# happyxtt/CNNs_SLFP_quantization

Hardware: AMD Instinct MI355X
Metric: images/sec at batch 256, MobileNetV1 SLFP<3,4> ImageNet-224; % HBM roofline (higher is better)
Workload: dtype f32 (1x1 contraction: fp16 MFMA operands, f32 accumulate); 1 GPU; mobilenetv1_imagenet224: all 27 Conv2d_Q layers, SLFP<3,4> Qbits=8, NHWC, batch 256 per GPU as 2 concurrent image groups of 128 on 2 HIP streams, inputs resident in HBM; batch_per_gpu=256, global_batch=256, parallelism=batch-sharded x1, one-time RCCL broadcast of the u8 weight codes, pointwise_mfma=pw_mfma_f16x1

## Files before the change

### cnns_slfp_quantization_amd/_lib.py

```python
import ctypes
import os

_HERE = os.path.dirname(os.path.abspath(__file__))
LIB_PATH = os.path.join(_HERE, "libslfp_hip.so")

OK, ERR_BAD_ARG, ERR_SHAPE, ERR_UNSUPPORTED, ERR_ALIGNMENT, ERR_HIP = 0, -1, -2, -3, -4, -5
FMT_ACT8, FMT_W8, FMT_SFP7, FMT_EXT = 0, 1, 2, 4
LAYOUT_NCHW, LAYOUT_NHWC = 0, 1
BWD_DENSE = 1
MFMA_DEFAULT, MFMA_F16X1, MFMA_F16X3 = 0, 1, 3
OPT_SGD, OPT_DSGD, OPT_SSGD = 0, 1, 2
LAYEROUT_LUT_BYTES = 4928

SYMBOLS = (
    "slfp_version", "slfp_last_error", "slfp_device_count",
    "slfp_encode_f32", "slfp_decode_f32", "slfp_quantize_f32", "slfp_quantize_layerout_f32", "slfp_absmax_f32",
    "slfp_conv2d_out_shape", "slfp_conv2d_kernel_name", "slfp_conv2d_wprep_bytes",
    "slfp_conv2d_prepare_weights", "slfp_conv2d_prepare_weights_codes", "slfp_conv2d_workspace_bytes", "slfp_conv2d_fwd", "slfp_conv2d_fwd_post",
    "slfp_linear_workspace_bytes", "slfp_linear_fwd", "slfp_linear_prepare_weights", "slfp_linear_fwd_prepared",
    "slfp_nchw_to_nhwc_f32", "slfp_nhwc_to_nchw_f32", "slfp_debug_div_mismatches",
    "slfp_debug_enc_mismatches", "slfp_enc_table_ok", "slfp_dwpw_supported", "slfp_dwpw_fwd",
    "slfp_conv2d_codes_supported", "slfp_conv2d_fwd_codes", "slfp_conv2d_fwd_codes_ws", "slfp_maxpool2d_codes", "slfp_debug_code_mismatches", "slfp_debug_reload_switches",
    "slfp_debug_enc_hl_mismatches", "slfp_sgd_step_f32", "slfp_debug_dw3x3_variant", "slfp_debug_dense_variant", "slfp_debug_pw_variant",
    "slfp_conv2d_bwd_supported", "slfp_conv2d_bwd_kernel_name", "slfp_conv2d_bwd_workspace_bytes", "slfp_conv2d_bwd",
    "slfp_conv2d_bwd_supported_ex", "slfp_conv2d_bwd_kernel_name_ex", "slfp_conv2d_bwd_workspace_bytes_ex", "slfp_conv2d_bwd_ex",
    "slfp_conv2d_res_supported", "slfp_conv2d_fwd_res",
    "slfp_conv2d_codes_slice_supported", "slfp_conv2d_fwd_codes_slice", "slfp_maxpool2d_codes_ex", "slfp_maxpool2d_out_shape",
    "slfp_conv2d_entry_supported", "slfp_conv2d_fwd_entry",
    "slfp_conv2d_res_codes_supported", "slfp_conv2d_fwd_res_codes",
    "slfp_layerout_lut_classes", "slfp_layerout_lut_values", "slfp_layerout_lut_index", "slfp_conv2d_codes_lut_supported",
    "slfp_conv2d_fwd_codes_lut", "slfp_debug_layerout_lut_mismatches",
    "slfp_dwpw_codes_supported", "slfp_dwpw_fwd_codes",
    "slfp_linear_fc_supported", "slfp_linear_fc_workspace_bytes", "slfp_linear_fwd_fc", "slfp_debug_linear_fc_tiles",
    "slfp_global_avgpool_supported", "slfp_global_avgpool_f32",
    "slfp_debug_dw3x3_instance", "slfp_debug_code_relu_mismatches",
    "slfp_bn_train_supported", "slfp_bn_train_workspace_bytes", "slfp_bn_train_fwd", "slfp_bn_train_bwd", "slfp_debug_bn_split",
    "slfp_debug_dwpw_instance",
)


class ConvDesc(ctypes.Structure):
    _fields_ = [
        ("n", ctypes.c_int64), ("c_in", ctypes.c_int64), ("h", ctypes.c_int64), ("w", ctypes.c_int64),
        ("c_out", ctypes.c_int64), ("kh", ctypes.c_int64), ("kw", ctypes.c_int64),
        ("stride_h", ctypes.c_int32), ("stride_w", ctypes.c_int32), ("pad_h", ctypes.c_int32),
        ("pad_w", ctypes.c_int32), ("dil_h", ctypes.c_int32), ("dil_w", ctypes.c_int32),
        ("groups", ctypes.c_int32), ("x_layout", ctypes.c_int32), ("y_layout", ctypes.c_int32),
        ("qbits", ctypes.c_int32), ("ka", ctypes.c_float), ("kw_scale", ctypes.c_float),
        ("mfma_passes", ctypes.c_int32), ("reserved", ctypes.c_int32),
    ]


class ConvIo(ctypes.Structure):
    _fields_ = [("x_codes", ctypes.c_int32), ("y_codes", ctypes.c_int32), ("y_ka", ctypes.c_float), ("y_qbits", ctypes.c_int32)]


class SgdHparams(ctypes.Structure):
    _fields_ = [("rule", ctypes.c_int32), ("qbits", ctypes.c_int32), ("lr", ctypes.c_float), ("momentum", ctypes.c_float),
                ("damp_alpha", ctypes.c_float), ("weight_decay", ctypes.c_float), ("nesterov", ctypes.c_int32),
                ("reserved", ctypes.c_int32)]


class SlfpError(RuntimeError):
    def __init__(self, code, text):
        super().__init__(f"libslfp_hip: {text} (status {code})")
        self.code = code


_lib = None


def load():
    global _lib
    if _lib is not None:
        return _lib
    if not os.path.exists(LIB_PATH):
        raise RuntimeError(
            f"{LIB_PATH} is missing: the SLFP HIP extension is not built. "
            "Run `python -m cnns_slfp_quantization_amd.build` (needs hipcc). There is no CPU fallback.")
    import torch
    L = ctypes.CDLL(LIB_PATH)
    vp, sz, ci, cf, i64 = ctypes.c_void_p, ctypes.c_size_t, ctypes.c_int, ctypes.c_float, ctypes.c_int64
    dp = ctypes.POINTER(ConvDesc)
    sigs = {
        "slfp_version": (ci, []),
        "slfp_last_error": (ctypes.c_char_p, []),
        "slfp_device_count": (ci, []),
        "slfp_encode_f32": (ci, [vp, vp, sz, cf, ci, vp]),
        "slfp_decode_f32": (ci, [vp, vp, sz, ci, vp]),
        "slfp_quantize_f32": (ci, [vp, vp, sz, cf, ci, vp]),
        "slfp_quantize_layerout_f32": (ci, [vp, vp, sz, vp]),
        "slfp_absmax_f32": (ci, [vp, sz, vp, vp]),
        "slfp_conv2d_out_shape": (ci, [dp, ctypes.POINTER(i64), ctypes.POINTER(i64)]),
        "slfp_conv2d_kernel_name": (ctypes.c_char_p, [dp]),
        "slfp_debug_dw3x3_variant": (ctypes.c_char_p, [dp, ci]),
        "slfp_debug_dw3x3_instance": (ctypes.c_char_p, [dp, ctypes.POINTER(ConvIo), ci, ci, ci]),
        "slfp_debug_code_relu_mismatches": (ci, [cf, ci, vp, vp]),
        "slfp_debug_dense_variant": (ctypes.c_char_p, [dp, ci]),
        "slfp_debug_pw_variant": (ctypes.c_char_p, [dp, ctypes.POINTER(ConvIo), ci, ci, i64]),
        "slfp_conv2d_wprep_bytes": (sz, [dp]),
        "slfp_conv2d_prepare_weights": (ci, [dp, vp, vp, vp, vp]),
        "slfp_conv2d_prepare_weights_codes": (ci, [dp, vp, vp, vp, vp]),
        "slfp_conv2d_workspace_bytes": (sz, [dp]),
        "slfp_conv2d_fwd": (ci, [dp, vp, vp, vp, vp, vp, vp, vp]),
        "slfp_conv2d_fwd_post": (ci, [dp, vp, vp, vp, vp, vp, ci, vp, vp, vp, vp]),
        "slfp_linear_workspace_bytes": (sz, [i64, i64, i64]),
        "slfp_linear_fwd": (ci, [vp, vp, vp, vp, i64, i64, i64, cf, cf, ci, ci, vp, vp]),
        "slfp_linear_prepare_weights": (ci, [vp, vp, i64, i64, cf, ci, ci, vp]),
        "slfp_linear_fwd_prepared": (ci, [vp, vp, vp, vp, i64, i64, i64, cf, cf, ci, ci, vp]),
        "slfp_nchw_to_nhwc_f32": (ci, [vp, vp, i64, i64, i64, i64, vp]),
        "slfp_nhwc_to_nchw_f32": (ci, [vp, vp, i64, i64, i64, i64, vp]),
        "slfp_debug_div_mismatches": (ci, [cf, vp, vp]),
        "slfp_debug_enc_mismatches": (ci, [cf, ci, vp, vp]),
        "slfp_enc_table_ok": (ci, [cf, ci]),
        "slfp_dwpw_supported": (ci, [dp, dp]),
        "slfp_dwpw_fwd": (ci, [dp, dp, vp, vp, vp, vp, ci, vp, vp, vp, vp, ci, vp, vp]),
        "slfp_conv2d_codes_supported": (ci, [dp, ctypes.POINTER(ConvIo), ci, ci]),
        "slfp_conv2d_fwd_codes": (ci, [dp, ctypes.POINTER(ConvIo), vp, vp, vp, vp, vp, ci, vp, vp]),
        "slfp_conv2d_fwd_codes_ws": (ci, [dp, ctypes.POINTER(ConvIo), vp, vp, vp, vp, vp, ci, vp, vp, vp]),
        "slfp_maxpool2d_codes": (ci, [vp, vp, i64, i64, i64, i64, ci, ci, ci, ci, ci, ci, ci, vp]),
        "slfp_debug_code_mismatches": (ci, [cf, ci, vp, vp]),
        "slfp_debug_reload_switches": (None, []),
        "slfp_debug_enc_hl_mismatches": (ci, [cf, ci, vp, vp]),
        "slfp_sgd_step_f32": (ci, [ctypes.POINTER(SgdHparams), sz, vp, vp, vp, vp, vp, vp]),
        "slfp_conv2d_bwd_supported": (ci, [dp]),
        "slfp_conv2d_bwd_kernel_name": (ctypes.c_char_p, [dp]),
        "slfp_conv2d_bwd_workspace_bytes": (sz, [dp, ci, ci]),
        "slfp_conv2d_bwd": (ci, [dp, vp, vp, vp, vp, vp, vp, vp, vp]),
        "slfp_conv2d_bwd_supported_ex": (ci, [dp, ctypes.c_uint]),
        "slfp_conv2d_bwd_kernel_name_ex": (ctypes.c_char_p, [dp, ctypes.c_uint]),
        "slfp_conv2d_bwd_workspace_bytes_ex": (sz, [dp, ctypes.c_uint, ci, ci]),
        "slfp_conv2d_bwd_ex": (ci, [dp, ctypes.c_uint, vp, vp, vp, vp, vp, vp, vp, vp]),
        "slfp_conv2d_res_supported": (ci, [dp, ctypes.POINTER(ConvIo), ci, ci]),
        "slfp_conv2d_fwd_res": (ci, [dp, ctypes.POINTER(ConvIo), vp, vp, vp, vp, vp, ci, vp, vp, vp, vp]),
        "slfp_conv2d_codes_slice_supported": (ci, [dp, ctypes.POINTER(ConvIo), ci, ci, i64]),
        "slfp_conv2d_fwd_codes_slice": (ci, [dp, ctypes.POINTER(ConvIo), vp, vp, vp, vp, vp, ci, vp, i64, vp, vp]),
        "slfp_maxpool2d_codes_ex": (ci, [vp, vp, i64, i64, i64, i64, ci, ci, ci, ci, ci, ci, ci, ci, vp]),
        "slfp_maxpool2d_out_shape": (ci, [i64, i64, ci, ci, ci, ci, ci, ci, ci, ctypes.POINTER(i64), ctypes.POINTER(i64)]),
        "slfp_conv2d_entry_supported": (ci, [dp, ctypes.POINTER(ConvIo), ci, ci]),
        "slfp_conv2d_fwd_entry": (ci, [dp, ctypes.POINTER(ConvIo), vp, vp, vp, vp, vp, ci, vp, vp]),
        "slfp_conv2d_res_codes_supported": (ci, [dp, ctypes.POINTER(ConvIo), ci, ci]),
        "slfp_conv2d_fwd_res_codes": (ci, [dp, ctypes.POINTER(ConvIo), vp, vp, vp, vp, vp, ci, vp, vp, vp, vp, vp]),
        "slfp_layerout_lut_classes": (ci, []),
        "slfp_layerout_lut_values": (ci, [vp, ci]),
        "slfp_layerout_lut_index": (ci, [cf]),
        "slfp_conv2d_codes_lut_supported": (ci, [dp, ctypes.POINTER(ConvIo), ci, i64]),
        "slfp_conv2d_fwd_codes_lut": (ci, [dp, ctypes.POINTER(ConvIo), vp, vp, vp, vp, vp, vp, vp, i64, vp, vp]),
        "slfp_debug_layerout_lut_mismatches": (ci, [vp, vp]),
# ... 36 lines not shown
```

### cnns_slfp_quantization_amd/csrc/codec.hip

```cpp
#include <cstdarg>
#include <mutex>
#include <map>
#include <set>
#include <utility>
#include <cstdio>
#include "slfp_device.hpp"
#include "slfp_enc.hpp"
#include "slfp_host.hpp"

namespace slfp {

static thread_local char g_err[512] = "";

void set_error(const char* fmt, ...) {
    va_list ap;
    va_start(ap, fmt);
    vsnprintf(g_err, sizeof(g_err), fmt, ap);
    va_end(ap);
}

int fail(int code, const char* fmt, ...) {
    va_list ap;
    va_start(ap, fmt);
    vsnprintf(g_err, sizeof(g_err), fmt, ap);
    va_end(ap);
    return code;
}

int check_launch(const char* what) {
    hipError_t e = hipGetLastError();
    if (e != hipSuccess) return fail(SLFP_ERR_HIP, "%s: %s", what, hipGetErrorString(e));
    return SLFP_OK;
}

const char* last_error_text() { return g_err; }

int raise_lds_limit(const void* fn, size_t lds_bytes) {
    if (lds_bytes <= 48 * 1024) return SLFP_OK;
    static std::mutex mu;
    static std::map<std::pair<int, const void*>, size_t> raised;
    int dev = 0;
    if (hipGetDevice(&dev) != hipSuccess) return check_launch("hipGetDevice");
    std::lock_guard<std::mutex> lock(mu);
    const auto key = std::make_pair(dev, fn);
    const auto it = raised.find(key);
    if (it != raised.end() && it->second >= lds_bytes) return SLFP_OK;
    if (hipFuncSetAttribute(fn, hipFuncAttributeMaxDynamicSharedMemorySize, (int)lds_bytes) != hipSuccess)
        return check_launch("hipFuncSetAttribute(MaxDynamicSharedMemorySize)");
    raised[key] = lds_bytes;
    return SLFP_OK;
}

static Switches read_switches() {
    Switches w;
    w.long_encode = std::getenv("SLFP_LONG_ENCODE") != nullptr;
    w.dw_old = std::getenv("SLFP_DW_OLD") != nullptr;
    w.pw_nostg = std::getenv("SLFP_PW_NOSTG") != nullptr;
    w.pw_notab = std::getenv("SLFP_PW_NOTAB") != nullptr;
    const char* e = std::getenv("SLFP_PW_STG_MAXKS");
    w.pw_stg_maxks = e ? atoi(e) : -1;
    e = std::getenv("SLFP_PW_NT_MIN_MB");
    w.pw_nt_min_mb = e ? atoll(e) : 0;
    e = std::getenv("SLFP_DW_NT_MIN_MB");
    w.dw_nt_min_mb = e ? atoll(e) : 30;
    w.stem_old = std::getenv("SLFP_STEM_OLD") != nullptr;
    w.pwc_slice = std::getenv("SLFP_PWC_NOSLICE") == nullptr;
    w.dense_generic = std::getenv("SLFP_DENSE_GENERIC") != nullptr;
    e = std::getenv("SLFP_DENSE_CFG");
    w.dense_cfg = e ? atoi(e) : 0;
    e = std::getenv("SLFP_DENSE_NWB");
    w.dense_nwb = e ? atoi(e) : 0;
    w.dense_res = std::getenv("SLFP_DENSE_NORES") == nullptr;
    w.dense_encx = std::getenv("SLFP_DENSE_NOENCX") == nullptr;
    w.stem_im2row = std::getenv("SLFP_STEM_IM2ROW") != nullptr;
    w.dw_rows = parse_dw_rows(std::getenv("SLFP_DW_ROWS"));
    e = std::getenv("SLFP_PW_GRID");
    w.pw_grid = e ? (atoi(e) > 0 ? atoi(e) : 0) : 0;
    e = std::getenv("SLFP_PW_STREAM_MAX_KB");
    w.pw_stream_max_kb = e ? atoi(e) : 30;
    return w;
}
static Switches g_switches = read_switches();
const Switches& switches() { return g_switches; }
void reload_switches() { g_switches = read_switches(); }

int device_cu_count() {
    static std::mutex mu;
    static std::map<int, int> cus;
    int dev = 0;
    if (hipGetDevice(&dev) != hipSuccess) { (void)hipGetLastError(); return 256; }
    std::lock_guard<std::mutex> lock(mu);
    const auto it = cus.find(dev);
    if (it != cus.end()) return it->second;
    int n = 0;
    if (hipDeviceGetAttribute(&n, hipDeviceAttributeMultiprocessorCount, dev) != hipSuccess || n <= 0) { (void)hipGetLastError(); n = 256; }
    cus[dev] = n;
    return n;
}

int resident_blocks_per_cu(const void* fn, int block_threads, size_t dynamic_lds) {
    static std::mutex mu;
    static std::map<std::pair<std::pair<int, const void*>, size_t>, int> cache;
    int dev = 0;
    if (hipGetDevice(&dev) != hipSuccess) { (void)hipGetLastError(); return 1; }
    const auto key = std::make_pair(std::make_pair(dev, fn), dynamic_lds);
    std::lock_guard<std::mutex> lock(mu);
    const auto it = cache.find(key);
    if (it != cache.end()) return it->second;
    int n = 0;
    if (hipOccupancyMaxActiveBlocksPerMultiprocessor(&n, fn, block_threads, dynamic_lds) != hipSuccess || n < 1) { (void)hipGetLastError(); n = 1; }
    cache[key] = n;
    return n;
}

constexpr int kThreads = 256;

template <int FMT, int MODE>
__global__ __launch_bounds__(kThreads) void k_codec(const float* __restrict__ x, void* __restrict__ out,
                                                    size_t n, const ScaleDiv sd, int ext, int vec_ok) {
    __shared__ uint32_t sT[16];
    lut_fill<FMT>(sT);
    __syncthreads();
    const size_t nvec = vec_ok ? n / 4 : 0;
    const size_t stride = (size_t)gridDim.x * kThreads;
    for (size_t i = (size_t)blockIdx.x * kThreads + threadIdx.x; i < nvec; i += stride) {
        const float4 v = reinterpret_cast<const float4*>(x)[i];
        const uint32_t u0 = __float_as_uint(div_const(v.x, sd)), u1 = __float_as_uint(div_const(v.y, sd));
        const uint32_t u2 = __float_as_uint(div_const(v.z, sd)), u3 = __float_as_uint(div_const(v.w, sd));
// ... 269 lines not shown
```

### cnns_slfp_quantization_amd/csrc/conv_abi.hip

```cpp
#include <cstring>
#include "slfp_device.hpp"
#include "slfp_codes.hpp"
#include "slfp_layerout_lut.hpp"
#include "slfp_host.hpp"

namespace slfp {

static size_t round256(size_t b) { return (b + 255) & ~(size_t)255; }

static int make_plan_core(const slfp_conv2d_desc* d, ConvPlan* plan) {
    if (!d || !plan) return fail(SLFP_ERR_BAD_ARG, "conv2d: null descriptor");
    if (d->n <= 0 || d->c_in <= 0 || d->h <= 0 || d->w <= 0 || d->c_out <= 0 || d->kh <= 0 || d->kw <= 0)
        return fail(SLFP_ERR_SHAPE, "conv2d: non-positive size");
    if (d->stride_h <= 0 || d->stride_w <= 0 || d->dil_h <= 0 || d->dil_w <= 0 || d->pad_h < 0 || d->pad_w < 0)
        return fail(SLFP_ERR_SHAPE, "conv2d: bad stride/dilation/padding");
    if (d->groups <= 0 || d->c_in % d->groups || d->c_out % d->groups)
        return fail(SLFP_ERR_SHAPE, "conv2d: groups=%d does not divide C_in=%lld / C_out=%lld", d->groups,
                    (long long)d->c_in, (long long)d->c_out);
    if (d->qbits != 8 && d->qbits != 7)
        return fail(SLFP_ERR_BAD_ARG, "conv2d: qbits must be 8 (SLFP<3,4>) or 7 (SFP<3,3>), got %d", d->qbits);
    if ((d->x_layout != SLFP_LAYOUT_NCHW && d->x_layout != SLFP_LAYOUT_NHWC) ||
        (d->y_layout != SLFP_LAYOUT_NCHW && d->y_layout != SLFP_LAYOUT_NHWC))
        return fail(SLFP_ERR_BAD_ARG, "conv2d: unknown layout");
    if (!(d->ka > 0.f) || !(d->kw_scale > 0.f)) return fail(SLFP_ERR_BAD_ARG, "conv2d: Ka and Kw must be > 0");
// ... 185 lines not shown
#undef SLFP_PREP
    return check_launch("slfp weight prepare kernel");
}

static const char* family_name(const ConvPlan& p, const slfp_conv2d_desc& d) {
    if (p.family == kDirect && stem_applicable(d)) return "stem_nhwc";
    if (p.repad) {
        if (p.family == kDw3x3) return "repad+dw3x3_nhwc";
        return p.fmt_act == kFmtSfp7 ? "repad+pw_mfma_f16_exact" : (p.passes == 3 ? "repad+pw_mfma_f16x3" : "repad+pw_mfma_f16x1");
    }
    switch (p.family) {
        case kDw3x3: return "dw3x3_nhwc";
        case kPointwise: return p.fmt_act == kFmtSfp7 ? "pw_mfma_f16_exact" : (p.passes == 3 ? "pw_mfma_f16x3" : "pw_mfma_f16x1");
        case kDenseMfma: return p.fmt_act == kFmtSfp7 ? "dense_mfma_f16_exact" : (p.passes == 3 ? "dense_mfma_f16x3" : "dense_mfma_f16x1");
        case kStemMfma: return p.fmt_act == kFmtSfp7 ? "stem_mfma_f16_exact" : "stem_mfma_f16x1";
        case kStemSmall: return p.fmt_act == kFmtSfp7 ? "stem_small_mfma_f16_exact" : "stem_small_mfma_f16x1";
        default: return "direct_nhwc";
    }
}

}

using namespace slfp;

static const char* pw_variant(const slfp_conv2d_desc* d, const slfp_conv2d_io* io, bool has_res, bool has_res_codes, int64_t y_ld);
static const char* dw3x3_instance(const slfp_conv2d_desc* d, const slfp_conv2d_io* io, bool has_bias, int post_flags, bool has_post);

extern "C" {

int slfp_conv2d_out_shape(const slfp_conv2d_desc* d, int64_t* h_out, int64_t* w_out) {
    ConvPlan p;
    const int rc = make_plan(d, &p);
    if (rc != SLFP_OK) return rc;
    if (h_out) *h_out = p.h_out;
    if (w_out) *w_out = p.w_out;
    return SLFP_OK;
}

const char* slfp_conv2d_kernel_name(const slfp_conv2d_desc* d) {
    ConvPlan p;
    if (make_plan(d, &p) != SLFP_OK) return "invalid";
    return family_name(p, *d);
}

const char* slfp_debug_dw3x3_variant(const slfp_conv2d_desc* d, int has_post) {
    ConvPlan p;
    if (make_plan(d, &p) != SLFP_OK || p.family != kDw3x3) return "none";
    static const float one = 1.f;
    const PostOp post = {has_post ? &one : nullptr, has_post ? &one : nullptr, 0, 0};
    if (dw3x3_rows_applicable(*d, p, nullptr, post)) return "rows";
    return dw3x3_tile_applicable(*d, p, nullptr, post) ? "tile" : "general";
}

const char* slfp_debug_dw3x3_instance(const slfp_conv2d_desc* d, const slfp_conv2d_io* io, int has_bias, int post_flags, int has_post) {
    return dw3x3_instance(d, io, has_bias != 0, post_flags, has_post != 0);
}

const char* slfp_debug_dense_variant(const slfp_conv2d_desc* d, int x_codes) {
    ConvPlan p;
    if (make_plan(d, &p) != SLFP_OK) return "none";
    return dense_variant_name(*d, p, x_codes != 0);
}

const char* slfp_debug_pw_variant(const slfp_conv2d_desc* d, const slfp_conv2d_io* io, int has_res, int has_res_codes, int64_t y_ld) {
    return pw_variant(d, io, has_res != 0, has_res_codes != 0, y_ld);
}

size_t slfp_conv2d_wprep_bytes(const slfp_conv2d_desc* d) {
    ConvPlan p;
    if (make_plan(d, &p) != SLFP_OK) return 0;
    return p.wprep_bytes;
}

static int prepare_weights(const char* fn, const slfp_conv2d_desc* d, const void* w, void* wprep, float* weight_q_oihw, void* stream,
                           bool codes) {
    ConvPlan p;
    const int rc = make_plan(d, &p);
    if (rc != SLFP_OK) return rc;
    if (!w || !wprep) return fail(SLFP_ERR_BAD_ARG, "%s: null pointer", fn);
    if (!aligned16(wprep)) return fail(SLFP_ERR_ALIGNMENT, "%s: wprep must be 16-byte aligned", fn);
    return launch_prepare_weights(*d, p, reinterpret_cast<const float*>(w), wprep, weight_q_oihw, as_stream(stream), codes);
}

int slfp_conv2d_prepare_weights(const slfp_conv2d_desc* d, const float* w_oihw, void* wprep, float* weight_q_oihw,
                                void* stream) {
    return prepare_weights("slfp_conv2d_prepare_weights", d, w_oihw, wprep, weight_q_oihw, stream, false);
}

int slfp_conv2d_prepare_weights_codes(const slfp_conv2d_desc* d, const uint8_t* codes_oihw, void* wprep, float* weight_q_oihw,
                                      void* stream) {
    return prepare_weights("slfp_conv2d_prepare_weights_codes", d, codes_oihw, wprep, weight_q_oihw, stream, true);
}

}

struct WsLayout {
    size_t x_nhwc, y_nhwc;
    size_t operand;
    size_t x_pad, y_pad;
    size_t vec[3];
    size_t total;
};

static WsLayout ws_layout(const slfp_conv2d_desc* d, const ConvPlan& p) {
    WsLayout l;
    size_t at = 0;
// ... 548 lines not shown
```

### cnns_slfp_quantization_amd/csrc/conv_dw2.hip

```cpp
#include <cstdlib>
#include "slfp_device.hpp"
#include "slfp_enc.hpp"
#include "slfp_host.hpp"

namespace slfp {

constexpr int kDw2Threads = 256;
constexpr int kDw2Tab = (kEncEntries * 8 + 15) & ~15;
constexpr uint32_t kOob = 0xFFFFFFF0u;

struct Dw2Params {
    int N, H, W, C, Ho, Wo;
    int tiles_h, tiles_w, cgroups;
    int pad;
    uint32_t ntiles;
    uint32_t nblocks;
    float ka, kw;
    int nt_out;
    PostOp post;
    EncArgs enc;
};

typedef float f32x4 __attribute__((ext_vector_type(4)));

__device__ __forceinline__ __amdgpu_buffer_rsrc_t make_rsrc(const void* base, uint32_t bytes) {
    return __builtin_amdgcn_make_buffer_rsrc(const_cast<void*>(base), 0, bytes, 0x00020000);
}

template <int S, int TH, int TW, bool POST>
__global__ __launch_bounds__(kDw2Threads, 4) void k_dw3x3_tile(const float* __restrict__ x, const float* __restrict__ wq,
                                                               float* __restrict__ y, const Dw2Params p) {
    constexpr int IH = (TH - 1) * S + 3, IW = (TW - 1) * S + 3;
    static_assert(IW <= 16 && IH <= 16, "halo tile is at most 16 x 16 pixel slots");
    constexpr int NI = (IH + 1) / 2;
    constexpr int ROWB = 16 * 32 * 4;

    __shared__ __attribute__((aligned(16))) unsigned char smem[kDw2Tab + 2 * NI * ROWB];
    unsigned char* tile = smem + kDw2Tab;
    enc_fill<kDw2Threads>(reinterpret_cast<uint2*>(smem), p.enc);
    const float r1 = p.enc.r1, lo = p.enc.lo, hi = p.enc.hi;

    const uint32_t lb = xcd_remap(blockIdx.x, p.nblocks);
    const int cg = (int)(lb % (uint32_t)p.cgroups);
    const uint32_t t = lb / (uint32_t)p.cgroups;

    const int c4 = threadIdx.x & 7, slot = threadIdx.x >> 3;
    const int c = cg * 32 + c4 * 4;
    const int iw = slot & 15, ihh = slot >> 4;

    f32x4 wt[9];
#pragma unroll
    for (int k = 0; k < 9; ++k) wt[k] = *reinterpret_cast<const f32x4*>(wq + (size_t)k * p.C + c);
    f32x4 psc = {1.f, 1.f, 1.f, 1.f}, psh = {0.f, 0.f, 0.f, 0.f};
    if constexpr (POST) {
        psc = *reinterpret_cast<const f32x4*>(p.post.scale + c);
        psh = *reinterpret_cast<const f32x4*>(p.post.shift + c);
    }

    const int colslot = (S == 2) ? ((iw & 1) * 8 + (iw >> 1)) : iw;
    const uint32_t lds_w = (uint32_t)((ihh * 16 + colslot) * 128 + c4 * 16);
    const bool col_live = iw < IW;
    constexpr int CW = TW > 8 ? 16 : 8, RPI = 32 / CW, NO = (TH + RPI - 1) / RPI;
    const int ow = slot & (CW - 1), ohb = slot / CW;
    const bool ocol_live = ow < TW;
    const uint32_t lds_r0 = (uint32_t)(((ohb * S) * 16 + ow) * 128 + c4 * 16);
    const uint32_t out_rel0 = (uint32_t)((ohb * p.Wo + ow) * p.C + c) * 4u;
    const uint32_t out_step = (uint32_t)(RPI * p.Wo * p.C) * 4u;
    const uint32_t img_in_bytes = (uint32_t)p.H * p.W * p.C * 4u, img_out_bytes = (uint32_t)p.Ho * p.Wo * p.C * 4u;
    const uint32_t tiles_per_img = (uint32_t)(p.tiles_h * p.tiles_w);
// ... 23 lines not shown
    }
    __syncthreads();

    bool any_nan = false;
#pragma unroll
    for (int i = 0; i < NI; ++i) {
        const float4 xi = make_float4(v[i][0], v[i][1], v[i][2], v[i][3]);
        any_nan |= enc_has_nan4(xi);
        *reinterpret_cast<float4*>(tile + lds_w + (uint32_t)i * 2u * ROWB) = enc4_f32_raw(xi, r1, lo, hi, smem);
    }
    if (__builtin_expect(any_nan, 0)) {
#pragma unroll
        for (int i = 0; i < NI; ++i)
#pragma unroll
            for (int e = 0; e < 4; ++e)
                if (v[i][e] != v[i][e]) reinterpret_cast<uint32_t*>(tile + lds_w + (uint32_t)i * 2u * ROWB)[e] = kBitsQNaN;
    }
    __syncthreads();

    const __amdgpu_buffer_rsrc_t ry = make_rsrc(y + (size_t)n * p.Ho * p.Wo * p.C, img_out_bytes);
    const int oh0 = th * TH, ow0 = tw * TW;
    const uint32_t org = (uint32_t)((oh0 * p.Wo + ow0) * p.C) * 4u;
#pragma unroll
    for (int j = 0; j < NO; ++j) {
        f32x4 acc = {0.f, 0.f, 0.f, 0.f};
#pragma unroll
        for (int kh = 0; kh < 3; ++kh) {
#pragma unroll
            for (int kw = 0; kw < 3; ++kw) {
                const int tap = j * RPI * S * ROWB + ((S == 1) ? (kh * ROWB + kw * 128) : (kh * ROWB + ((kw & 1) * 8 + (kw >> 1)) * 128));
                const f32x4 a = *reinterpret_cast<const f32x4*>(tile + lds_r0 + tap);
                const f32x4 w = wt[kh * 3 + kw];
#pragma unroll
                for (int e = 0; e < 4; ++e) acc[e] = fmaf(a[e], w[e], acc[e]);
            }
        }
        f32x4 rr;
#pragma unroll
        for (int e = 0; e < 4; ++e) {
            float u = (acc[e] * p.ka) * p.kw;
            if constexpr (POST) u = __builtin_fmaf(u, psc[e], psh[e]);
            if (p.post.relu) u = fmaxf(u, 0.f);
            rr[e] = u;
        }
        const bool live = ocol_live && (oh0 + ohb + j * RPI) < p.Ho && (j * RPI + ohb) < TH && (ow0 + ow) < p.Wo;
        uint32_t so = live ? org + out_rel0 + (uint32_t)j * out_step : kOob;
        asm volatile("" : "+v"(so));
        typedef unsigned int u32x4s __attribute__((ext_vector_type(4)));
        if (p.nt_out) __builtin_amdgcn_raw_buffer_store_b128(__builtin_bit_cast(u32x4s, rr), ry, so, 0, 2);
        else __builtin_amdgcn_raw_buffer_store_b128(__builtin_bit_cast(u32x4s, rr), ry, so, 0, 0);
    }
}

bool dw3x3_tile_applicable(const slfp_conv2d_desc& d, const ConvPlan& plan, const float* bias, const PostOp& post) {
    if (bias) return false;
    if (long_encode_forced() || dw_old_forced()) return false;
    if (plan.family != kDw3x3 || plan.repad) return false;
    if (d.c_in % 32 != 0 || post.layerout) return false;
    if (d.pad_h > 2) return false;
    if (d.stride_h == 1 && plan.h_out <= 7 && plan.w_out <= 7) return false;
    if ((int64_t)d.h * d.w * d.c_in >= (1ll << 29) || plan.h_out * plan.w_out * d.c_in >= (1ll << 29)) return false;
    return act_table(d.ka, plan.fmt_act, kEncF32) != nullptr;
}

struct Dw2Sel { int s; bool post; };
static Dw2Sel dw2_select(const slfp_conv2d_desc& d, const PostOp& post) { return Dw2Sel{d.stride_h == 2 ? 2 : 1, post.scale != nullptr}; }

const char* dw3x3_tile_name(const slfp_conv2d_desc& d, const ConvPlan& plan, const PostOp& post) {
    const Dw2Sel s = dw2_select(d, post);
    if (s.s == 2) return s.post ? "tile/s2/post" : "tile/s2/plain";
    return s.post ? "tile/s1/post" : "tile/s1/plain";
}

int launch_dw3x3_tile(const slfp_conv2d_desc& d, const ConvPlan& plan, const float* x, const float* wq9c,
                      const PostOp& post, float* y, hipStream_t stream) {
    Dw2Params p;
    const Dw2Sel sel = dw2_select(d, post);
    p.post = post;
    p.N = (int)d.n; p.H = (int)d.h; p.W = (int)d.w; p.C = (int)d.c_in;
    p.Ho = (int)plan.h_out; p.Wo = (int)plan.w_out;
    const int S = sel.s;
    const int TH = S == 2 ? 7 : 14, TW = TH;
    p.tiles_h = (int)ceil_div(p.Ho, TH);
    p.tiles_w = (int)ceil_div(p.Wo, TW);
    p.cgroups = p.C / 32;
    p.pad = d.pad_h;
    const int64_t ntiles = (int64_t)p.N * p.tiles_h * p.tiles_w;
    if (ntiles * p.cgroups > 0x7FFFFFFF) return fail(SLFP_ERR_UNSUPPORTED, "dw3x3: grid too large");
    p.ntiles = (uint32_t)ntiles;
    p.nblocks = (uint32_t)(ntiles * p.cgroups);
    p.ka = d.ka; p.kw = d.kw_scale;
    {
        const int64_t min_mb = switches().dw_nt_min_mb;
        p.nt_out = ((SLFP_NT_DW & 2) && (int64_t)p.N * p.Ho * p.Wo * p.C * 4 >= (min_mb << 20)) ? 1 : 0;
    }
    p.enc = *act_table(d.ka, plan.fmt_act, kEncF32);
#define SLFP_DW2(SS, TT) \
    do { if (sel.post) hipLaunchKernelGGL((k_dw3x3_tile<SS, TT, TT, true>), dim3(p.nblocks), dim3(kDw2Threads), 0, stream, x, wq9c, y, p); \
         else hipLaunchKernelGGL((k_dw3x3_tile<SS, TT, TT, false>), dim3(p.nblocks), dim3(kDw2Threads), 0, stream, x, wq9c, y, p); } while (0)
    if (S == 2) SLFP_DW2(2, 7);
    else SLFP_DW2(1, 14);
#undef SLFP_DW2
    return check_launch("slfp dw3x3 (tile) kernel");
}

}
```

### cnns_slfp_quantization_amd/csrc/slfp_host.hpp

```cpp
#pragma once
#include <hip/hip_runtime.h>
#include <stdint.h>
#include <stddef.h>
#include <cmath>
#include <cstring>
#include <cstdlib>
#include "../../include/slfp.h"
#include "slfp_device.hpp"
#include "slfp_enc.hpp"

namespace slfp {

void set_error(const char* fmt, ...);
int fail(int code, const char* fmt, ...);
int check_launch(const char* what);

int raise_lds_limit(const void* fn, size_t lds_bytes);

inline hipStream_t as_stream(void* s) { return reinterpret_cast<hipStream_t>(s); }
inline bool aligned16(const void* p) { return (reinterpret_cast<uintptr_t>(p) & 15u) == 0; }
inline int64_t ceil_div(int64_t a, int64_t b) { return (a + b - 1) / b; }

inline bool scale_div_ok(float d) { return std::isfinite(d) && d >= 1e-30f && d <= 1e30f; }

inline ScaleDiv make_scale_div(float d, int esh = 0) {
    ScaleDiv s;
    s.d = std::ldexp(d, -esh);
    s.r = (float)(1.0 / (double)s.d);
    return s;
}

struct Switches {
    bool long_encode, dw_old, pw_nostg, pw_notab;
    int pw_stg_maxks;
    long long pw_nt_min_mb;
    long long dw_nt_min_mb;
    bool stem_old;
    bool pwc_slice;
    bool dense_generic;
    int dense_cfg;
    int dense_nwb;
    bool dense_encx;
    bool dense_res;
    bool stem_im2row;
    int dw_rows;
    int pw_grid;
    int pw_stream_max_kb;
};
const Switches& switches();
void reload_switches();
inline bool long_encode_forced() { return switches().long_encode; }
inline bool dw_old_forced() { return switches().dw_old; }
inline const EncArgs* act_table(float ka, int fmt_act, int rep) {
    if (long_encode_forced()) return nullptr;
    const EncArgs* t = enc_table(ka, fmt_act, rep);
    return t->valid ? t : nullptr;
}

enum KernelFamily { kDw3x3 = 0, kPointwise = 1, kDirect = 2, kDenseMfma = 3, kStemMfma = 4, kStemSmall = 5 };

struct ConvPlan {
    KernelFamily family;
    int fmt_act;
    int fmt_w;
    int passes;
    int64_t h_out, w_out;
    float s1, s2;
    int64_t k_pad, n_pad;
    size_t wprep_bytes;
    bool repad;
    int64_t cpi, cpo;
};

int make_plan(const slfp_conv2d_desc* d, ConvPlan* plan);

int launch_quantize(const float* x, float* y, size_t n, float scale, int fmt, hipStream_t stream);
int launch_dw3x3(const slfp_conv2d_desc& d, const ConvPlan& p, const float* x, const float* wq9c,
                 const float* bias, const PostOp& post, float* y, hipStream_t stream);
bool dw3x3_tile_applicable(const slfp_conv2d_desc& d, const ConvPlan& p, const float* bias, const PostOp& post);
int launch_dw3x3_tile(const slfp_conv2d_desc& d, const ConvPlan& p, const float* x, const float* wq9c,
                      const PostOp& post, float* y, hipStream_t stream);
bool dw3x3_rows_applicable(const slfp_conv2d_desc& d, const ConvPlan& p, const float* bias, const PostOp& post);
int launch_dw3x3_rows(const slfp_conv2d_desc& d, const ConvPlan& p, const float* x, const float* wq9c,
                      const PostOp& post, float* y, hipStream_t stream);
const char* dw3x3_instance_name(const slfp_conv2d_desc& d, const ConvPlan& p, bool has_bias, const PostOp& post);
const char* dw3x3_tile_name(const slfp_conv2d_desc& d, const ConvPlan& p, const PostOp& post);
const char* dw3x3_rows_name(const slfp_conv2d_desc& d, const ConvPlan& p, const PostOp& post);
inline int parse_dw_rows(const char* e) {
    if (!e || !*e) return -1;
    const long v = strtol(e, nullptr, 0);
    return v <= 0 ? 0 : (int)(v & 0xF);
}
inline int dw_rows_class(int64_t h_out, int64_t w_out) {
    const int64_t px = h_out * w_out;
    return px >= 56 * 56 ? 0 : (px >= 28 * 28 ? 1 : (px >= 14 * 14 ? 2 : 3));
}
int launch_pointwise(const slfp_conv2d_desc& d, const ConvPlan& p, const float* x, const void* wfrag,
                     const float* bias, const PostOp& post, float* y, hipStream_t stream, const float* res = nullptr);
bool pointwise_res_applicable(const slfp_conv2d_desc& d, const ConvPlan& p);
const char* pw_variant_name(const slfp_conv2d_desc& d, const ConvPlan& p, bool has_res, bool y_codes, float y_ka, int y_fmt);
struct CodeIo {
    bool x_codes;
    bool y_codes;
    float y_ka;
    int y_fmt;
    int64_t y_ld = 0;
    const uint8_t* lut = nullptr;
};
int resident_blocks_per_cu(const void* fn, int block_threads, size_t dynamic_lds);
int device_cu_count();
bool pointwise_entry_applicable(const slfp_conv2d_desc& d, const ConvPlan& p, int post_flags, float y_ka, int y_fmt);
int launch_pointwise_entry(const slfp_conv2d_desc& d, const ConvPlan& p, const float* x, const void* wfrag, const float* bias,
                           const PostOp& post, void* y_codes, const CodeIo& io, hipStream_t stream);
bool pwc_applicable(const slfp_conv2d_desc& d, const ConvPlan& p, int post_flags, bool y_codes);
int launch_pwc(const slfp_conv2d_desc& d, const ConvPlan& p, const uint8_t* x, const void* wfrag, const float* bias,
               const PostOp& post, void* y, const CodeIo& io, hipStream_t stream, const float* res = nullptr, void* res_codes = nullptr);
const char* pwc_variant_name(const slfp_conv2d_desc& d, const ConvPlan& p, bool y_codes, bool has_res, bool has_dual, bool lut = false);
bool stem_codes_applicable(const slfp_conv2d_desc& d, const ConvPlan& p, int post_flags);
int launch_stem_codes(const slfp_conv2d_desc& d, const ConvPlan& p, const float* x, const float* wq_hwio, const float* bias,
                      const PostOp& post, void* y, const CodeIo& io, hipStream_t stream);
bool dwc_applicable(const slfp_conv2d_desc& d, const ConvPlan& p, const float* bias, int post_flags);
int launch_dwc(const slfp_conv2d_desc& d, const ConvPlan& p, const uint8_t* x, const float* wq9c, const PostOp& post,
               void* y, const CodeIo& io, hipStream_t stream);
const char* dwc_instance_name(const slfp_conv2d_desc& d, const ConvPlan& p, const PostOp& post, const CodeIo& io);
#define SLFP_DWPW_INSTANCES(X)                                                                                   \
    X(1, 1, 4) X(1, 1, 8) X(1, 1, 16) X(1, 2, 4) X(1, 2, 8) X(1, 2, 16) X(1, 4, 4) X(1, 4, 8) X(1, 4, 16)        \
    X(2, 1, 4) X(2, 1, 8) X(2, 1, 16) X(2, 2, 4) X(2, 2, 8) X(2, 2, 16) X(2, 4, 4) X(2, 4, 8) X(2, 4, 16)
struct DwPwSel {
    int s, ks, nt;
    int fmt_in;
    bool yc;
};
inline bool dwpw_instance_built(int s, int ks, int nt) {
#define SLFP_DWPW_HAS(SS, KK, NN) if (s == SS && ks == KK && nt == NN) return true;
    SLFP_DWPW_INSTANCES(SLFP_DWPW_HAS)
#undef SLFP_DWPW_HAS
    return false;
}
bool dwpw_select(const slfp_conv2d_desc* dw, const slfp_conv2d_desc* pw, DwPwSel* s);
bool dwpw_codes_select(const slfp_conv2d_desc* dw, const slfp_conv2d_desc* pw, const slfp_conv2d_io* io, int relu1, int relu2, DwPwSel* s);
int launch_direct(const slfp_conv2d_desc& d, const ConvPlan& p, const float* x, const float* wq_hwio,
                  const float* bias, const PostOp& post, float* y, hipStream_t stream);
bool stem_applicable(const slfp_conv2d_desc& d);
bool pointwise_stream_fits(int64_t k_pad, int64_t n_pad, int passes);
// ... 39 lines not shown
```

### include/slfp.h

```cpp
#ifndef SLFP_H_
#define SLFP_H_

#include <stddef.h>
#include <stdint.h>

#ifdef __cplusplus
extern "C" {
#endif

#define SLFP_ABI_VERSION 1

#define SLFP_OK 0
#define SLFP_ERR_BAD_ARG (-1)
#define SLFP_ERR_SHAPE (-2)
#define SLFP_ERR_UNSUPPORTED (-3)
#define SLFP_ERR_ALIGNMENT (-4)
#define SLFP_ERR_HIP (-5)

#define SLFP_FMT_ACT8 0
#define SLFP_FMT_W8 1
#define SLFP_FMT_SFP7 2
#define SLFP_FMT_EXT 4

#define SLFP_LAYOUT_NCHW 0
#define SLFP_LAYOUT_NHWC 1

#define SLFP_MFMA_DEFAULT 0
#define SLFP_MFMA_F16X1 1
#define SLFP_MFMA_F16X3 3

int slfp_version(void);
void slfp_debug_reload_switches(void);
const char* slfp_last_error(void);
int slfp_device_count(void);


int slfp_encode_f32(const float* x, uint8_t* code, size_t n, float scale_div, int fmt, void* stream);
int slfp_decode_f32(const uint8_t* code, float* y, size_t n, int fmt, void* stream);
int slfp_quantize_f32(const float* x, float* y, size_t n, float scale_div, int fmt, void* stream);

int slfp_quantize_layerout_f32(const float* x, float* y, size_t n, void* stream);
int slfp_absmax_f32(const float* x, size_t n, float* out, void* stream);


typedef struct slfp_conv2d_desc {
    int64_t n, c_in, h, w;
    int64_t c_out, kh, kw;
    int32_t stride_h, stride_w, pad_h, pad_w, dil_h, dil_w, groups;
    int32_t x_layout, y_layout;
    int32_t qbits;
    float ka, kw_scale;
    int32_t mfma_passes;
    int32_t reserved;
} slfp_conv2d_desc;

int slfp_conv2d_out_shape(const slfp_conv2d_desc* d, int64_t* h_out, int64_t* w_out);
const char* slfp_conv2d_kernel_name(const slfp_conv2d_desc* d);
const char* slfp_debug_dw3x3_variant(const slfp_conv2d_desc* d, int has_post);
const char* slfp_debug_dense_variant(const slfp_conv2d_desc* d, int x_codes);
struct slfp_conv2d_io;
const char* slfp_debug_dw3x3_instance(const slfp_conv2d_desc* d, const struct slfp_conv2d_io* io, int has_bias, int post_flags, int has_post);
const char* slfp_debug_pw_variant(const slfp_conv2d_desc* d, const struct slfp_conv2d_io* io, int has_res, int has_res_codes, int64_t y_ld);

size_t slfp_conv2d_wprep_bytes(const slfp_conv2d_desc* d);
int slfp_conv2d_prepare_weights(const slfp_conv2d_desc* d, const float* w_oihw, void* wprep,
                                float* weight_q_oihw, void* stream);
int slfp_conv2d_prepare_weights_codes(const slfp_conv2d_desc* d, const uint8_t* codes_oihw, void* wprep,
                                      float* weight_q_oihw, void* stream);
size_t slfp_conv2d_workspace_bytes(const slfp_conv2d_desc* d);
int slfp_conv2d_fwd(const slfp_conv2d_desc* d, const float* x, const void* wprep, const float* bias,
                    float* y, float* input_q, void* workspace, void* stream);

#define SLFP_POST_RELU 1
#define SLFP_POST_LAYEROUT 2
int slfp_conv2d_fwd_post(const slfp_conv2d_desc* d, const float* x, const void* wprep, const float* bias,
                         const float* post_scale, const float* post_shift, int relu, float* y,
                         float* input_q, void* workspace, void* stream);

int slfp_dwpw_supported(const slfp_conv2d_desc* dw, const slfp_conv2d_desc* pw);
int slfp_dwpw_fwd(const slfp_conv2d_desc* dw, const slfp_conv2d_desc* pw, const float* x, const void* wprep_dw,
                  const float* post1_scale, const float* post1_shift, int relu1, const void* wprep_pw,
                  const float* bias_pw, const float* post2_scale, const float* post2_shift, int relu2, float* y,
                  void* stream);

typedef struct slfp_conv2d_io {
    int32_t x_codes;
    int32_t y_codes;
    float y_ka;
    int32_t y_qbits;
} slfp_conv2d_io;
int slfp_conv2d_codes_supported(const slfp_conv2d_desc* d, const slfp_conv2d_io* io, int has_bias, int relu);
int slfp_conv2d_fwd_codes(const slfp_conv2d_desc* d, const slfp_conv2d_io* io, const void* x, const void* wprep,
                          const float* bias, const float* post_scale, const float* post_shift, int relu, void* y,
                          void* stream);
int slfp_conv2d_fwd_codes_ws(const slfp_conv2d_desc* d, const slfp_conv2d_io* io, const void* x, const void* wprep,
                             const float* bias, const float* post_scale, const float* post_shift, int relu, void* y,
                             void* workspace, void* stream);
int slfp_dwpw_codes_supported(const slfp_conv2d_desc* dw, const slfp_conv2d_desc* pw, const slfp_conv2d_io* io,
                              int has_bias_pw, int relu1, int relu2);
int slfp_dwpw_fwd_codes(const slfp_conv2d_desc* dw, const slfp_conv2d_desc* pw, const slfp_conv2d_io* io, const void* x,
                        const void* wprep_dw, const float* post1_scale, const float* post1_shift, int relu1,
                        const void* wprep_pw, const float* bias_pw, const float* post2_scale, const float* post2_shift,
                        int relu2, void* y, void* stream);
const char* slfp_debug_dwpw_instance(const slfp_conv2d_desc* dw, const slfp_conv2d_desc* pw, const slfp_conv2d_io* io,
                                     int has_bias_pw, int relu1, int relu2);
int slfp_conv2d_codes_slice_supported(const slfp_conv2d_desc* d, const slfp_conv2d_io* io, int has_bias, int relu, int64_t y_ld);
int slfp_conv2d_fwd_codes_slice(const slfp_conv2d_desc* d, const slfp_conv2d_io* io, const void* x, const void* wprep,
                                const float* bias, const float* post_scale, const float* post_shift, int relu, void* y,
                                int64_t y_ld, void* workspace, void* stream);
int slfp_conv2d_entry_supported(const slfp_conv2d_desc* d, const slfp_conv2d_io* io, int has_bias, int relu);
int slfp_conv2d_fwd_entry(const slfp_conv2d_desc* d, const slfp_conv2d_io* io, const float* x, const void* wprep,
// ... 100 lines not shown
```

Measured before the change: 132,100 images/sec.

## Add register-window body for stride-1 depthwise 3x3 tile kernel

Adds a new stride-1 depthwise 3x3 kernel in which each wave streams input rows through a register ring with prefetch depth 2-3. Horizontal neighbours are exchanged with ds_bpermute instead of an LDS tile, and rolling accumulators emit each output row as soon as it is complete. The aim is to remove LDS staging and barrier cost in the tile path for the largest spatial class (56x56) by default, with 7- or 14-row bodies selectable via SLFP_DW_WIN. In exchange it needs more registers per thread and does more redundant halo encoding per wave.

```diff
diff --git a/cnns_slfp_quantization_amd/_lib.py b/cnns_slfp_quantization_amd/_lib.py
--- a/cnns_slfp_quantization_amd/_lib.py
+++ b/cnns_slfp_quantization_amd/_lib.py
@@ -33,7 +33,7 @@
     "slfp_dwpw_codes_supported", "slfp_dwpw_fwd_codes",
     "slfp_linear_fc_supported", "slfp_linear_fc_workspace_bytes", "slfp_linear_fwd_fc", "slfp_debug_linear_fc_tiles",
     "slfp_global_avgpool_supported", "slfp_global_avgpool_f32",
-    "slfp_debug_dw3x3_instance", "slfp_debug_code_relu_mismatches",
+    "slfp_debug_dw3x3_instance", "slfp_debug_dw3x3_tile_body", "slfp_debug_code_relu_mismatches",
     "slfp_bn_train_supported", "slfp_bn_train_workspace_bytes", "slfp_bn_train_fwd", "slfp_bn_train_bwd", "slfp_debug_bn_split",
     "slfp_debug_dwpw_instance",
 )
@@ -94,6 +94,7 @@
         "slfp_conv2d_out_shape": (ci, [dp, ctypes.POINTER(i64), ctypes.POINTER(i64)]),
         "slfp_conv2d_kernel_name": (ctypes.c_char_p, [dp]),
         "slfp_debug_dw3x3_variant": (ctypes.c_char_p, [dp, ci]),
+        "slfp_debug_dw3x3_tile_body": (ctypes.c_char_p, [dp, ci]),
         "slfp_debug_dw3x3_instance": (ctypes.c_char_p, [dp, ctypes.POINTER(ConvIo), ci, ci, ci]),
         "slfp_debug_code_relu_mismatches": (ci, [cf, ci, vp, vp]),
         "slfp_debug_dense_variant": (ctypes.c_char_p, [dp, ci]),
diff --git a/cnns_slfp_quantization_amd/csrc/codec.hip b/cnns_slfp_quantization_amd/csrc/codec.hip
--- a/cnns_slfp_quantization_amd/csrc/codec.hip
+++ b/cnns_slfp_quantization_amd/csrc/codec.hip
@@ -74,6 +74,7 @@
     w.dense_encx = std::getenv("SLFP_DENSE_NOENCX") == nullptr;
     w.stem_im2row = std::getenv("SLFP_STEM_IM2ROW") != nullptr;
     w.dw_rows = parse_dw_rows(std::getenv("SLFP_DW_ROWS"));
+    w.dw_win = parse_dw_win(std::getenv("SLFP_DW_WIN"));
     e = std::getenv("SLFP_PW_GRID");
     w.pw_grid = e ? (atoi(e) > 0 ? atoi(e) : 0) : 0;
     e = std::getenv("SLFP_PW_STREAM_MAX_KB");
diff --git a/cnns_slfp_quantization_amd/csrc/conv_abi.hip b/cnns_slfp_quantization_amd/csrc/conv_abi.hip
--- a/cnns_slfp_quantization_amd/csrc/conv_abi.hip
+++ b/cnns_slfp_quantization_amd/csrc/conv_abi.hip
@@ -261,6 +261,15 @@
     return dw3x3_tile_applicable(*d, p, nullptr, post) ? "tile" : "general";
 }
 
+const char* slfp_debug_dw3x3_tile_body(const slfp_conv2d_desc* d, int has_post) {
+    ConvPlan p;
+    if (make_plan(d, &p) != SLFP_OK || p.family != kDw3x3) return "none";
+    static const float one = 1.f;
+    const PostOp post = {has_post ? &one : nullptr, has_post ? &one : nullptr, 0, 0};
+    if (dw3x3_rows_applicable(*d, p, nullptr, post) || !dw3x3_tile_applicable(*d, p, nullptr, post)) return "none";
+    return dw3x3_tile_body_name(*d, p);
+}
+
 const char* slfp_debug_dw3x3_instance(const slfp_conv2d_desc* d, const slfp_conv2d_io* io, int has_bias, int post_flags, int has_post) {
     return dw3x3_instance(d, io, has_bias != 0, post_flags, has_post != 0);
 }
diff --git a/cnns_slfp_quantization_amd/csrc/conv_dw2.hip b/cnns_slfp_quantization_amd/csrc/conv_dw2.hip
--- a/cnns_slfp_quantization_amd/csrc/conv_dw2.hip
+++ b/cnns_slfp_quantization_amd/csrc/conv_dw2.hip
@@ -15,6 +15,7 @@
     int pad;
     uint32_t ntiles;
     uint32_t nblocks;
+    uint32_t nwin_blocks;
     float ka, kw;
     int nt_out;
     PostOp post;
@@ -144,6 +145,142 @@
     }
 }
 
+constexpr int kDw2WinWaves = kDw2Threads / 64;
+
+template <bool POST, bool NT, int TH>
+__global__ __launch_bounds__(kDw2Threads, 4) void k_dw3x3_tile_win(const float* __restrict__ x, const float* __restrict__ wq,
+                                                                   float* __restrict__ y, const Dw2Params p) {
+    constexpr int T = 14, NR = TH + 2;
+    constexpr int DEPTH = POST ? 2 : 3;
+    typedef unsigned int u32x4w __attribute__((ext_vector_type(4)));
+
+    __shared__ __attribute__((aligned(16))) unsigned char smem[kDw2Tab];
+    enc_fill<kDw2Threads>(reinterpret_cast<uint2*>(smem), p.enc);
+    const float r1 = p.enc.r1, lo = p.enc.lo, hi = p.enc.hi;
+
+    uint32_t t = xcd_remap(blockIdx.x, p.nwin_blocks) * kDw2WinWaves + (uint32_t)__builtin_amdgcn_readfirstlane((int)(threadIdx.x >> 6));
+    const bool valid = t < p.nblocks;
+    t = valid ? t : p.nblocks - 1;
+    const int cg = (int)(t % (uint32_t)p.cgroups); t /= (uint32_t)p.cgroups;
+    const int tw = (int)(t % (uint32_t)p.tiles_w); t /= (uint32_t)p.tiles_w;
+    const int th = (int)(t % (uint32_t)p.tiles_h);
+    const int n = (int)(t / (uint32_t)p.tiles_h);
+    const int lane = (int)(threadIdx.x & 63), g = lane >> 3;
+    const int c = cg * 32 + (lane & 7) * 4;
+
+    f32x4 wt[9];
+#pragma unroll
+    for (int k = 0; k < 9; ++k) wt[k] = *reinterpret_cast<const f32x4*>(wq + (uint32_t)(k * p.C + c));
+    f32x4 psc = {1.f, 1.f, 1.f, 1.f}, psh = {0.f, 0.f, 0.f, 0.f};
+    if constexpr (POST) {
+        psc = *reinterpret_cast<const f32x4*>(p.post.scale + c);
+        psh = *reinterpret_cast<const f32x4*>(p.post.shift + c);
+    }
+
+    const uint32_t img_in = (uint32_t)(p.H * p.W * p.C) * 4u, img_out = (uint32_t)(p.Ho * p.Wo * p.C) * 4u;
+    const __amdgpu_buffer_rsrc_t rs = make_rsrc(x + (size_t)n * (img_in / 4u), img_in);
+    const __amdgpu_buffer_rsrc_t ry = make_rsrc(y + (size_t)n * (img_out / 4u), img_out);
+
+    const int ih0 = valid ? th * TH - p.pad : -0x40000000;
+    const int iw0 = tw * T - p.pad + 2 * g;
+    const uint32_t rstep = (uint32_t)(p.W * p.C) * 4u;
+    const uint32_t rowb = (uint32_t)ih0 * rstep + (uint32_t)c * 4u;
+    uint32_t coff[2];
+#pragma unroll
+    for (int k = 0; k < 2; ++k) coff[k] = (unsigned)(iw0 + k) < (unsigned)p.W ? (uint32_t)((iw0 + k) * p.C) * 4u : 0x40000000u;
+    const int left_addr = ((lane - 8) & 63) * 4, right_addr = ((lane + 8) & 63) * 4;
+
+    f32x4 raw[DEPTH][2];
+    auto request = [&](const int j) {
+        const uint32_t roff = (unsigned)(ih0 + j) < (unsigned)p.H ? rowb + (uint32_t)j * rstep : 0x80000000u;
+#pragma unroll
+        for (int k = 0; k < 2; ++k)
+            raw[j % DEPTH][k] = __builtin_bit_cast(f32x4, __builtin_amdgcn_raw_buffer_load_b128(rs, roff + coff[k], 0, (SLFP_NT_DW & 1) ? 2 : 0));
+    };
+#pragma unroll
+    for (int j = 0; j < DEPTH; ++j) request(j);
+
+    const int oh0 = th * TH;
+    const uint32_t ostep = (uint32_t)(p.Wo * p.C) * 4u;
+    uint32_t ocol[2];
+#pragma unroll
+    for (int k = 0; k < 2; ++k) {
+        const int ow = tw * T + 2 * g - 1 + k;
+        const bool live = valid && (k == 0 ? g > 0 : g < 7) && ow < p.Wo;
+        ocol[k] = live ? (uint32_t)((oh0 * p.Wo + ow) * p.C + c) * 4u : 0x80000000u;
+    }
+
+    __syncthreads();
+
+    f32x4 acc[3][2];
+#pragma unroll
+    for (int j = 0; j < NR; ++j) {
+        f32x4 win[4];
+        {
+            const f32x4 v0 = raw[j % DEPTH][0], v1 = raw[j % DEPTH][1];
+            bool any_nan = enc_has_nan4(make_float4(v0[0], v0[1], v0[2], v0[3]));
+            any_nan |= enc_has_nan4(make_float4(v1[0], v1[1], v1[2], v1[3]));
+            uint32_t nan_mask = 0;
+            if (__builtin_expect(any_nan, 0)) {
+#pragma unroll
+                for (int e = 0; e < 4; ++e) {
+                    if (v0[e] != v0[e]) nan_mask |= 1u << e;
+                    if (v1[e] != v1[e]) nan_mask |= 16u << e;
+                }
+            }
+            const float4 q0 = enc4_f32_raw(make_float4(v0[0], v0[1], v0[2], v0[3]), r1, lo, hi, smem);
+            const float4 q1 = enc4_f32_raw(make_float4(v1[0], v1[1], v1[2], v1[3]), r1, lo, hi, smem);
+            win[1] = f32x4{q0.x, q0.y, q0.z, q0.w};
+            win[2] = f32x4{q1.x, q1.y, q1.z, q1.w};
+            if (__builtin_expect(nan_mask != 0, 0)) {
+#pragma unroll
+                for (int e = 0; e < 4; ++e) {
+                    if (nan_mask >> e & 1u) win[1][e] = __uint_as_float(kBitsQNaN);
+                    if (nan_mask >> (4 + e) & 1u) win[2][e] = __uint_as_float(kBitsQNaN);
+                }
+            }
+        }
+        if (j + DEPTH < NR) request(j + DEPTH);
+#pragma unroll
+        for (int e = 0; e < 4; ++e) {
+            win[0][e] = __int_as_float(__builtin_amdgcn_ds_bpermute(left_addr, __float_as_int(win[2][e])));
+            win[3][e] = __int_as_float(__builtin_amdgcn_ds_bpermute(right_addr, __float_as_int(win[1][e])));
+        }
+#pragma unroll
+        for (int kh = 2; kh >= 0; --kh) {
+            const int r = j - kh;
+            if (r < 0 || r >= TH) continue;
+#pragma unroll
+            for (int k = 0; k < 2; ++k) {
+                f32x4 a = {0.f, 0.f, 0.f, 0.f};
+                if (kh != 0) a = acc[r % 3][k];
+#pragma unroll
+                for (int kw = 0; kw < 3; ++kw) {
+                    const f32x4 v = win[k + kw];
+                    const f32x4 w = wt[kh * 3 + kw];
+#pragma unroll
+                    for (int e = 0; e < 4; ++e) a[e] = fmaf(v[e], w[e], a[e]);
+                }
+                acc[r % 3][k] = a;
+            }
+            if (kh != 2) continue;
+            const uint32_t orow = (oh0 + r) < p.Ho ? (uint32_t)r * ostep : 0x40000000u;
+#pragma unroll
+            for (int k = 0; k < 2; ++k) {
+                f32x4 rr;
+#pragma unroll
+                for (int e = 0; e < 4; ++e) {
+                    float u = (acc[r % 3][k][e] * p.ka) * p.kw;
+                    if constexpr (POST) u = __builtin_fmaf(u, psc[e], psh[e]);
+                    if (p.post.relu) u = fmaxf(u, 0.f);
+                    rr[e] = u;
+                }
+                __builtin_amdgcn_raw_buffer_store_b128(__builtin_bit_cast(u32x4w, rr), ry, ocol[k] + orow, 0, NT ? 2 : 0);
+            }
+        }
+    }
+}
+
 bool dw3x3_tile_applicable(const slfp_conv2d_desc& d, const ConvPlan& plan, const float* bias, const PostOp& post) {
     if (bias) return false;
     if (long_encode_forced() || dw_old_forced()) return false;
@@ -162,6 +299,22 @@
     const Dw2Sel s = dw2_select(d, post);
     if (s.s == 2) return s.post ? "tile/s2/post" : "tile/s2/plain";
     return s.post ? "tile/s1/post" : "tile/s1/plain";
+}
+
+constexpr int kDw2WinRule = 0x11;
+
+static int dw2_window_body(const slfp_conv2d_desc& d, const ConvPlan& plan) {
+    const int sw = switches().dw_win;
+    if (sw == 0 || d.stride_h != 1 || d.stride_w != 1 || d.pad_h != d.pad_w) return 0;
+    if ((int64_t)d.h * d.w * d.c_in * 4 > (1ll << 30) || plan.h_out * plan.w_out * d.c_in * 4 > (1ll << 30)) return 0;
+    const int rule = (sw < 0) ? kDw2WinRule : sw, cls = dw_rows_class(plan.h_out, plan.w_out);
+    if (!((rule >> cls) & 1)) return 0;
+    return ((rule >> (4 + cls)) & 1) ? 7 : 14;
+}
+
+const char* dw3x3_tile_body_name(const slfp_conv2d_desc& d, const ConvPlan& plan) {
+    const int rows = dw2_window_body(d, plan);
+    return rows == 0 ? "lds" : (rows == 7 ? "window/half" : "window");
 }
 
 int launch_dw3x3_tile(const slfp_conv2d_desc& d, const ConvPlan& plan, const float* x, const float* wq9c,
@@ -187,6 +340,21 @@
         p.nt_out = ((SLFP_NT_DW & 2) && (int64_t)p.N * p.Ho * p.Wo * p.C * 4 >= (min_mb << 20)) ? 1 : 0;
     }
     p.enc = *act_table(d.ka, plan.fmt_act, kEncF32);
+    p.nwin_blocks = 0;
+    if (const int rows = S == 1 ? dw2_window_body(d, plan) : 0) {
+        p.tiles_h = (int)ceil_div(p.Ho, rows);
+        const int64_t ntasks = (int64_t)p.N * p.tiles_h * p.tiles_w * p.cgroups;
+        if (ntasks > 0x7FFFFFFF) return fail(SLFP_ERR_UNSUPPORTED, "dw3x3: grid too large");
+        p.nblocks = (uint32_t)ntasks;
+        p.nwin_blocks = (uint32_t)ceil_div(ntasks, kDw2WinWaves);
+#define SLFP_DW2_WIN(PP, NN) \
+    do { if (rows == 7) hipLaunchKernelGGL((k_dw3x3_tile_win<PP, NN, 7>), dim3(p.nwin_blocks), dim3(kDw2Threads), 0, stream, x, wq9c, y, p); \
+         else hipLaunchKernelGGL((k_dw3x3_tile_win<PP, NN, 14>), dim3(p.nwin_blocks), dim3(kDw2Threads), 0, stream, x, wq9c, y, p); } while (0)
+        if (sel.post) { if (p.nt_out) SLFP_DW2_WIN(true, true); else SLFP_DW2_WIN(true, false); }
+        else { if (p.nt_out) SLFP_DW2_WIN(false, true); else SLFP_DW2_WIN(false, false); }
+#undef SLFP_DW2_WIN
+        return check_launch("slfp dw3x3 (tile, window body) kernel");
+    }
 #define SLFP_DW2(SS, TT) \
     do { if (sel.post) hipLaunchKernelGGL((k_dw3x3_tile<SS, TT, TT, true>), dim3(p.nblocks), dim3(kDw2Threads), 0, stream, x, wq9c, y, p); \
          else hipLaunchKernelGGL((k_dw3x3_tile<SS, TT, TT, false>), dim3(p.nblocks), dim3(kDw2Threads), 0, stream, x, wq9c, y, p); } while (0)
diff --git a/cnns_slfp_quantization_amd/csrc/slfp_host.hpp b/cnns_slfp_quantization_amd/csrc/slfp_host.hpp
--- a/cnns_slfp_quantization_amd/csrc/slfp_host.hpp
+++ b/cnns_slfp_quantization_amd/csrc/slfp_host.hpp
@@ -44,6 +44,7 @@
     bool dense_res;
     bool stem_im2row;
     int dw_rows;
+    int dw_win;
     int pw_grid;
     int pw_stream_max_kb;
 };
@@ -86,10 +87,16 @@
 const char* dw3x3_instance_name(const slfp_conv2d_desc& d, const ConvPlan& p, bool has_bias, const PostOp& post);
 const char* dw3x3_tile_name(const slfp_conv2d_desc& d, const ConvPlan& p, const PostOp& post);
 const char* dw3x3_rows_name(const slfp_conv2d_desc& d, const ConvPlan& p, const PostOp& post);
+const char* dw3x3_tile_body_name(const slfp_conv2d_desc& d, const ConvPlan& p);
 inline int parse_dw_rows(const char* e) {
     if (!e || !*e) return -1;
     const long v = strtol(e, nullptr, 0);
     return v <= 0 ? 0 : (int)(v & 0xF);
+}
+inline int parse_dw_win(const char* e) {
+    if (!e || !*e) return -1;
+    const long v = strtol(e, nullptr, 0);
+    return v <= 0 ? 0 : (int)(v & 0xFF);
 }
 inline int dw_rows_class(int64_t h_out, int64_t w_out) {
     const int64_t px = h_out * w_out;
diff --git a/include/slfp.h b/include/slfp.h
--- a/include/slfp.h
+++ b/include/slfp.h
@@ -57,6 +57,7 @@
 int slfp_conv2d_out_shape(const slfp_conv2d_desc* d, int64_t* h_out, int64_t* w_out);
 const char* slfp_conv2d_kernel_name(const slfp_conv2d_desc* d);
 const char* slfp_debug_dw3x3_variant(const slfp_conv2d_desc* d, int has_post);
+const char* slfp_debug_dw3x3_tile_body(const slfp_conv2d_desc* d, int has_post);
 const char* slfp_debug_dense_variant(const slfp_conv2d_desc* d, int x_codes);
 struct slfp_conv2d_io;
 const char* slfp_debug_dw3x3_instance(const slfp_conv2d_desc* d, const struct slfp_conv2d_io* io, int has_bias, int post_flags, int has_post);
```

Result: slower. 127,900 images/sec (-3.2%).
